# FatimaSohailll/KLT-Feature-Tracker-Acceleration-GPUs

Hardware: NVIDIA B200
Metric: tracked_features_per_s (higher is better)
Workload: dtype f32

## Files before the change

klt-feature-tracker-acceleration-gpus_b200/csrc/klt_dev.cu:

```cuda
#include <cuda_runtime.h>
#include <cub/device/device_radix_sort.cuh>
#include <cub/device/device_select.cuh>
#include <thrust/iterator/counting_iterator.h>
#include <climits>

#include <cstdarg>
#include <cstdio>
#include <cstdlib>
#include <cstring>
#include <sched.h>

#include "klt_cuda.h"

#define KLT_TRACKED         0
#define KLT_NOT_FOUND      -1
#define KLT_SMALL_DET      -2
#define KLT_MAX_ITERATIONS -3
#define KLT_OOB            -4
#define KLT_LARGE_RESIDUE  -5
#define KLT_B200_FB_INCONSISTENT -6

template <bool EXACT>
__device__ __forceinline__ float mac(float acc, float a, float b) {
  if (EXACT) return __fadd_rn(acc, __fmul_rn(a, b));
// ... 1117 lines not shown
  const unsigned char* src; int spitch;
  klt_dev_build_desc desc;
};

struct klt_dev {
  int device, num_sms;
  cudaStream_t stream;
  cudaStream_t tstream;
  cudaStream_t stream2;
  int overlap;
  cudaEvent_t ev_built[KLT_DEV_SLOTS];
  cudaEvent_t ev_read[KLT_DEV_SLOTS];
  int read_pending[KLT_DEV_SLOTS], built_pending[KLT_DEV_SLOTS];
  cudaEvent_t ev_join;
  char err[512];
  unsigned long long launches;
  int last_path, force_generic, no_fused, last_fused, track7_off;
  int W, H, L, ss;
  PyrSet set[KLT_DEV_SLOTS];
  float* arena;
  size_t arena_floats;
  int guard;
  struct Guarded { void* user; size_t bytes; } guarded[24]; int nguarded;
  float* tmp;
  unsigned char* frame;
  unsigned char* frame_buf[2]; int frame_idx;
  size_t frame_cap; int frame_pitch;
  cudaStream_t cstream;
  cudaEvent_t ev_band[KLT_BAND_EVENTS]; int band_ev_next;
  cudaEvent_t ev_frame_free[2]; int frame_busy[2];
  int band_rows, last_bands, building_slot;
  unsigned char* h_frame; size_t h_frame_cap; cudaEvent_t ev_stage_free; int stage_busy, stage_threads, last_staged;
  struct HostReg { const void* p; size_t bytes; int seen; int registered; unsigned long long stamp; } hreg[KLT_HOST_REGS];
  int reg_frames; unsigned long long reg_clock; int last_registered;
  int pdl;
  float *d_x, *d_y; int* d_val; int feat_cap; int feat_n;
  float *h_x, *h_y; int* h_val;
  int staging_busy;
  int no_track7w;
  int feat_out_host;
  unsigned char* d_rec; size_t d_rec_cap; void* h_rec; int rec_stride;
  cudaEvent_t ev_feat; int feat_pending;
  int feat_deferred; void* feat_def_dst; const void* feat_def_src; size_t feat_def_bytes;
  AffState* d_aff_st; AffState* h_aff_st; float* d_aff_tmpl; float* d_x0; int aff_cap, aff_tsz, aff_x0_cap;
  unsigned char* snap_ring; size_t snap_bytes; int snap_depth, snap_events; cudaEvent_t ev_snap[KLT_SNAP_MAX];
  int *c_val[2]; unsigned* c_idx[2]; size_t cand_cap;
  void* cub_tmp; size_t cub_bytes;
  unsigned char* fmap; size_t fmap_cap;
  int* open_slots; int open_cap;
  int* rank_list; int* sel_state;
  int no_filter; int replace_filter;
  int enforce_attr;
  unsigned* d_tile_ctr; unsigned tile_base[KLT_TILE_QUEUES];
  cudaEvent_t ev_a, ev_b; int ev_made;
  int prof_on, prof_used;
  cudaEvent_t* prof_ev;
  int* prof_kid;
  double prof_ms[KID_COUNT];
  unsigned long long prof_n[KID_COUNT];
  cudaEvent_t ev_origin;
  int trace_n; int* trace_kid; float* trace_t0; float* trace_t1;
  unsigned long long* d_live;
  FbRec* d_fb; int fb_cap, fb_n; float fb_max_error;
  PredVel* d_vel; PredRec* d_pred; int pred_cap, pred_n, vel_n;
  float* d_guess; float* h_guess; int guess_cap, guess_n, guess_slot;
  cudaEvent_t ev_guess[2]; int guess_busy[2];
  PredArgs pred;
};

static void prof_fold(klt_dev* d) {
  if (d->prof_used == 0) return;
  cudaStreamSynchronize(d->stream);
  if (d->stream2) cudaStreamSynchronize(d->stream2);
  if (d->cstream) cudaStreamSynchronize(d->cstream);
  for (int i = 0; i < d->prof_used; ++i) {
    float ms = 0.0f;
    if (cudaEventElapsedTime(&ms, d->prof_ev[2 * i], d->prof_ev[2 * i + 1]) == cudaSuccess) {
      d->prof_ms[d->prof_kid[i]] += ms;
      d->prof_n[d->prof_kid[i]] += 1;
      if (d->trace_n < TRACE_CAP) {
        float t0 = 0.0f;
        cudaEventElapsedTime(&t0, d->ev_origin, d->prof_ev[2 * i]);
        d->trace_kid[d->trace_n] = d->prof_kid[i];
        d->trace_t0[d->trace_n] = t0; d->trace_t1[d->trace_n] = t0 + ms;
        d->trace_n += 1;
      }
    }
  }
  d->prof_used = 0;
}
static int sync_all(klt_dev* d) {
  cudaError_t e = cudaStreamSynchronize(d->stream);
  if (e == cudaSuccess && d->stream2) e = cudaStreamSynchronize(d->stream2);
  if (e == cudaSuccess && d->cstream) e = cudaStreamSynchronize(d->cstream);
  d->staging_busy = 0;
  return e == cudaSuccess ? 0 : 1;
}
struct Launch {
  klt_dev* d; int slot; cudaStream_t st;
  Launch(klt_dev* d_, int kid, cudaStream_t st_ = nullptr) : d(d_), slot(-1), st(st_ ? st_ : d_->stream) {
    if (kid != KID_COPY_H2D && kid != KID_COPY_D2H) d->launches++;
    if (d->prof_on) {
      if (d->prof_used == PROF_POOL) prof_fold(d);
      slot = d->prof_used++;
      d->prof_kid[slot] = kid;
      cudaEventRecord(d->prof_ev[2 * slot], st);
// ... 136 lines not shown

static constexpr size_t KLT_GUARD_FLOATS = 1024;
static constexpr int KLT_GUARD_BYTE = 0xA5;
static cudaError_t guarded_malloc(klt_dev* d, void** out, size_t bytes) {
  if (!d->guard || d->nguarded >= (int)(sizeof(d->guarded) / sizeof(d->guarded[0]))) return cudaMalloc(out, bytes);
  const size_t gb = KLT_GUARD_FLOATS * sizeof(float), padded = (bytes + 255) / 256 * 256;
  unsigned char* base = nullptr;
  cudaError_t e = cudaMalloc(&base, padded + 2 * gb);
  if (e != cudaSuccess) return e;
  e = cudaMemset(base, KLT_GUARD_BYTE, padded + 2 * gb);
  if (e != cudaSuccess) { cudaFree(base); return e; }
  *out = base + gb;
  d->guarded[d->nguarded].user = base + gb; d->guarded[d->nguarded].bytes = bytes; d->nguarded += 1;
  return cudaSuccess;
}
template <typename T>
static cudaError_t guarded_malloc(klt_dev* d, T** out, size_t bytes) { return guarded_malloc(d, reinterpret_cast<void**>(out), bytes); }
static void guarded_free(klt_dev* d, void* p) {
  if (!p) return;
  for (int i = 0; i < d->nguarded; ++i)
    if (d->guarded[i].user == p) {
      cudaFree(static_cast<unsigned char*>(p) - KLT_GUARD_FLOATS * sizeof(float));
      d->guarded[i] = d->guarded[--d->nguarded];
      return;
    }
  cudaFree(p);
}
static void free_geometry(klt_dev* d) {
  cudaFree(d->arena); d->arena = nullptr;
  cudaFree(d->tmp); d->tmp = nullptr;
  memset(d->set, 0, sizeof(d->set));
  d->W = d->H = d->L = d->ss = 0;
}

extern "C" void klt_dev_destroy(klt_dev* d) {
  if (!d) return;
  cudaSetDevice(d->device);
  sync_all(d);
  klt_dev_forget_host_frames(d);
  free_geometry(d);
  cudaFree(d->frame_buf[0]); cudaFree(d->frame_buf[1]);
  guarded_free(d, d->d_x);
  guarded_free(d, d->d_fb);
  guarded_free(d, d->d_vel); guarded_free(d, d->d_pred); guarded_free(d, d->d_guess); cudaFreeHost(d->h_guess);
  for (int i = 0; i < 2; ++i) if (d->ev_guess[i]) cudaEventDestroy(d->ev_guess[i]);
  cudaFreeHost(d->h_x);
  for (int i = 0; i < 2; ++i) { guarded_free(d, d->c_val[i]); guarded_free(d, d->c_idx[i]); }
  cudaFree(d->cub_tmp); guarded_free(d, d->fmap); guarded_free(d, d->open_slots); guarded_free(d, d->rank_list); guarded_free(d, d->sel_state);
  if (d->ev_made) { cudaEventDestroy(d->ev_a); cudaEventDestroy(d->ev_b); }
  if (d->prof_ev) { for (int i = 0; i < 2 * PROF_POOL; ++i) cudaEventDestroy(d->prof_ev[i]); free(d->prof_ev); free(d->prof_kid);
    cudaEventDestroy(d->ev_origin); free(d->trace_kid); free(d->trace_t0); free(d->trace_t1); }
  cudaFree(d->d_live);
  cudaFree(d->d_tile_ctr);
  cudaFree(d->d_rec);
  for (int i = 0; i < KLT_DEV_SLOTS; ++i) { cudaEventDestroy(d->ev_built[i]); cudaEventDestroy(d->ev_read[i]); }
  cudaEventDestroy(d->ev_join);
  for (int i = 0; i < KLT_BAND_EVENTS; ++i) cudaEventDestroy(d->ev_band[i]);
  cudaEventDestroy(d->ev_frame_free[0]); cudaEventDestroy(d->ev_frame_free[1]);
  cudaEventDestroy(d->ev_feat);
  cudaEventDestroy(d->ev_stage_free);
  cudaFreeHost(d->h_frame);
  cudaFreeHost(d->snap_ring);
  cudaFree(d->d_aff_st); cudaFreeHost(d->h_aff_st); cudaFree(d->d_aff_tmpl); cudaFree(d->d_x0);
  for (int i = 0; i < d->snap_events; ++i) cudaEventDestroy(d->ev_snap[i]);
  cudaStreamDestroy(d->cstream);
  cudaStreamDestroy(d->stream);
  cudaStreamDestroy(d->stream2);
  free(d);
}

static int ensure_geometry(klt_dev* d, int W, int H, int L, int ss) {
  if (d->arena && d->W == W && d->H == H && d->L == L && d->ss == ss) return 0;
  if (W <= 0 || H <= 0) return fail(d, "bad image size %d x %d", W, H);
  if (L < 1 || L > KLT_DEV_MAX_LEVELS) return fail(d, "nPyramidLevels %d not in 1..%d", L, KLT_DEV_MAX_LEVELS);
  if (L > 1 && ss != 2 && ss != 4 && ss != 8 && ss != 16 && ss != 32)
    return fail(d, "Pyramid's subsampling must be either 2, 4, 8, 16, or 32");
  if (sync_all(d)) return fail(d, "stream synchronisation failed");
  memset(d->read_pending, 0, sizeof(d->read_pending));
  memset(d->built_pending, 0, sizeof(d->built_pending));
  free_geometry(d);
  d->vel_n = 0;
  size_t per_set = 0;
  int w = W, h = H;
  int ws[KLT_DEV_MAX_LEVELS], hs[KLT_DEV_MAX_LEVELS], ps[KLT_DEV_MAX_LEVELS];
  for (int l = 0; l < L; ++l) {
    ws[l] = w; hs[l] = h; ps[l] = (w + 31) / 32 * 32;
    if (w < 1 || h < 1) return fail(d, "pyramid level %d is empty (%d x %d)", l, w, h);
    per_set += 3 * (size_t)ps[l] * h;
    if (L > 1) { w /= ss; h /= ss; }
  }
  const size_t gap = d->guard ? KLT_GUARD_FLOATS : 0;
  const size_t total = KLT_DEV_SLOTS * (per_set + 3 * (size_t)L * gap) + gap;
  CU(cudaMalloc(&d->arena, total * sizeof(float) + 256));
  d->arena_floats = total;
  if (d->guard) CU(cudaMemset(d->arena, KLT_GUARD_BYTE, total * sizeof(float) + 256));
  CU(cudaMalloc(&d->tmp, (size_t)ps[0] * H * sizeof(float)));
  float* p = d->arena;
  for (int s = 0; s < KLT_DEV_SLOTS; ++s)
    for (int l = 0; l < L; ++l) {
      Level& lv = d->set[s].lv[l];
      lv.w = ws[l]; lv.h = hs[l]; lv.pitch = ps[l];
      const size_t n = (size_t)ps[l] * hs[l];
      p += gap; lv.img = p; p += n; p += gap; lv.gx = p; p += n; p += gap; lv.gy = p; p += n;
    }
  d->W = W; d->H = H; d->L = L; d->ss = ss;
  return 0;
}

extern "C" void klt_dev_set_guard(klt_dev* d, int on) {
  if (d->guard == (on ? 1 : 0)) return;
  sync_all(d);
  free_geometry(d);
  for (int i = 0; i < 2; ++i) { guarded_free(d, d->c_val[i]); guarded_free(d, d->c_idx[i]); d->c_val[i] = nullptr; d->c_idx[i] = nullptr; }
  guarded_free(d, d->rank_list); guarded_free(d, d->sel_state); d->rank_list = nullptr; d->sel_state = nullptr;
  cudaFree(d->cub_tmp); d->cub_tmp = nullptr; d->cand_cap = 0;
  guarded_free(d, d->fmap); d->fmap = nullptr; d->fmap_cap = 0;
  guarded_free(d, d->open_slots); d->open_slots = nullptr; d->open_cap = 0;
  d->guard = on ? 1 : 0;
}
extern "C" int klt_dev_check_guards(klt_dev* d, long long* damaged_words, int* first_band) {
  if (damaged_words) *damaged_words = 0;
  if (first_band) *first_band = -1;
  if (!d->guard) return 0;
  CU(cudaSetDevice(d->device));
  if (sync_all(d)) return fail(d, "stream synchronisation failed");
  unsigned* h = (unsigned*)malloc(KLT_GUARD_FLOATS * sizeof(unsigned));
  if (!h) return fail(d, "out of memory");
  const unsigned want = 0x01010101u * (unsigned)KLT_GUARD_BYTE;
  long long bad = 0;
  int first = -1, band = 0;
  auto check = [&](const float* at) -> int {
    if (cudaMemcpy(h, at, KLT_GUARD_FLOATS * sizeof(unsigned), cudaMemcpyDeviceToHost) != cudaSuccess) return 1;
    for (size_t i = 0; i < KLT_GUARD_FLOATS; ++i)
      if (h[i] != want) { bad += 1; if (first < 0) first = band; }
    band += 1;
    return 0;
  };
  int rc = 0;
  for (int s = 0; d->arena && s < KLT_DEV_SLOTS && !rc; ++s)
    for (int l = 0; l < d->L && !rc; ++l) {
      const Level& lv = d->set[s].lv[l];
      rc = check(lv.img - KLT_GUARD_FLOATS) || check(lv.gx - KLT_GUARD_FLOATS) || check(lv.gy - KLT_GUARD_FLOATS);
    }
  if (!rc && d->arena) rc = check(d->arena + d->arena_floats - KLT_GUARD_FLOATS);
  band = 1000;
  for (int i = 0; i < d->nguarded && !rc; ++i) {
    const unsigned char* u = static_cast<const unsigned char*>(d->guarded[i].user);
    rc = check(reinterpret_cast<const float*>(u - KLT_GUARD_FLOATS * sizeof(float))) ||
         check(reinterpret_cast<const float*>(u + (d->guarded[i].bytes + 255) / 256 * 256));
  }
  free(h);
  if (rc) return fail(d, "guard check: copy failed");
  if (damaged_words) *damaged_words = bad;
  if (first_band) *first_band = first;
  return 0;
}

extern "C" void* klt_dev_plane_address(const klt_dev* d, int slot, int which, int level) {
  if (!d->arena || slot < 0 || slot >= KLT_DEV_SLOTS || level < 0 || level >= d->L) return nullptr;
  const Level& lv = d->set[slot].lv[level];
  return which == 0 ? (void*)lv.img : which == 1 ? (void*)lv.gx : which == 2 ? (void*)lv.gy : nullptr;
}
extern "C" int klt_dev_poke(klt_dev* d, void* device_dst, const void* host_src, size_t bytes) {
  CU(cudaSetDevice(d->device));
  if (sync_all(d)) return fail(d, "stream synchronisation failed");
  CU(cudaMemcpy(device_dst, host_src, bytes, cudaMemcpyHostToDevice));
  return 0;
}

extern "C" int klt_dev_geometry(const klt_dev* d, int* W, int* H, int* L, int* ss) {
// ... 96 lines not shown
  { Launch l(d, KID_PYRDOWN);
    pyrdown_tile<SS, R, TXO, TYO, PY, EXACT><<<grid, NT, smem, d->stream>>>(src, spitch, W, H, t, out,
                                                                           opitch, Wout, Hout); }
  return 0;
}
template <bool EXACT>
static int pyrdown_dispatch(klt_dev* d, int ss, const float* src, int spitch, int W, int H,
                            const TapsR& t, float* out, int opitch, int Wout, int Hout, bool* done) {
  *done = true;
  const int r = t.w / 2;
  if (ss == 2 && r == 5) return launch_pyrdown<2, 5, 32, 32, 4, EXACT>(d, src, spitch, W, H, t, out, opitch, Wout, Hout);
  if (ss == 4 && r == 10) return launch_pyrdown<4, 10, 32, 16, 2, EXACT>(d, src, spitch, W, H, t, out, opitch, Wout, Hout);
  *done = false;
  return 0;
}

typedef CUresult (*EncodeTiledFn)(CUtensorMap*, CUtensorMapDataType, cuuint32_t, void*, const cuuint64_t*,
                                  const cuuint64_t*, const cuuint32_t*, const cuuint32_t*,
                                  CUtensorMapInterleave, CUtensorMapSwizzle, CUtensorMapL2promotion,
                                  CUtensorMapFloatOOBfill);
static EncodeTiledFn tma_encoder() {
  static EncodeTiledFn fn = nullptr;
  static bool tried = false;
  if (!tried) {
    tried = true;
    void* p = nullptr;
    cudaDriverEntryPointQueryResult q;
    if (cudaGetDriverEntryPoint("cuTensorMapEncodeTiled", &p, cudaEnableDefault, &q) == cudaSuccess &&
        q == cudaDriverEntryPointSuccess)
      fn = (EncodeTiledFn)p;
    cudaGetLastError();
  }
  return fn;
}
static bool make_tensor_map(CUtensorMap* m, const void* base, CUtensorMapDataType dt, int elem, int w, int h,
                            size_t pitch_bytes, int box_w, int box_h) {
  EncodeTiledFn enc = tma_encoder();
  if (!enc) return false;
  if (((uintptr_t)base & 15) || (pitch_bytes & 15) || ((box_w * elem) & 15) || box_w > 256 || box_h > 256)
    return false;
  cuuint64_t dims[2] = {(cuuint64_t)w, (cuuint64_t)h};
  cuuint64_t strides[1] = {(cuuint64_t)pitch_bytes};
  cuuint32_t box[2] = {(cuuint32_t)box_w, (cuuint32_t)box_h};
  cuuint32_t estr[2] = {1, 1};
  return enc(m, dt, 2, const_cast<void*>(base), dims, strides, box, estr, CU_TENSOR_MAP_INTERLEAVE_NONE,
             CU_TENSOR_MAP_SWIZZLE_NONE, CU_TENSOR_MAP_L2_PROMOTION_L2_128B,
             CU_TENSOR_MAP_FLOAT_OOB_FILL_NONE) == CUDA_SUCCESS;
}

static bool fused_grad_taps_ok(const TapsR& tg, const TapsR& td) {
  return tg.w == 2 * FUSED_RG + 1 && td.w == 2 * FUSED_RG + 1 && td.k[FUSED_RG] == 0.0f;
}

enum LevelShape { SHAPE_NONE = 0, SHAPE_2_5_64_32, SHAPE_2_5_64_16, SHAPE_2_5_32_16, SHAPE_4_10_32_16 };
struct FusedPlan {
  bool l0_ok;
  int shape[KLT_DEV_MAX_LEVELS];
  CUtensorMap map[KLT_DEV_MAX_LEVELS];
  int TX[KLT_DEV_MAX_LEVELS], TY[KLT_DEV_MAX_LEVELS], tiles_x[KLT_DEV_MAX_LEVELS], tiles_y[KLT_DEV_MAX_LEVELS];
  bool l0_march;
  bool chain;
  int src_plane[KLT_DEV_MAX_LEVELS], need_mul[KLT_DEV_MAX_LEVELS], need_add[KLT_DEV_MAX_LEVELS],
      made_mul[KLT_DEV_MAX_LEVELS];
};

static int level_shape_for(int ss, int r, int w, int h, int num_sms) {
  if (ss == 2 && r == 5) {
    const long px = (long)w * h;
    const long tiles_64x32 = (long)((w + 63) / 64) * ((h + 31) / 32);
    if (px >= 1500000) return SHAPE_2_5_64_32;
    if (px >= 300000) return tiles_64x32 <= 2L * num_sms ? SHAPE_2_5_64_32 : SHAPE_2_5_64_16;
    return SHAPE_2_5_32_16;
  }
  if (ss == 4 && r == 10) return SHAPE_4_10_32_16;
  return SHAPE_NONE;
}
template <int SS_, int R_, int TX_, int TY_>
struct TileShape { static constexpr int SS = SS_, R = R_, TX = TX_, TY = TY_; };
template <class F>
static auto with_shape(int shape, F f) {
  switch (shape) {
    case SHAPE_2_5_64_32: return f(TileShape<2, 5, 64, 32>());
    case SHAPE_2_5_64_16: return f(TileShape<2, 5, 64, 16>());
    case SHAPE_2_5_32_16: return f(TileShape<2, 5, 32, 16>());
    default: return f(TileShape<4, 10, 32, 16>());
  }
}

using L0GeoB = L0GeoT<48, 6, 6, 4>;
using L0GeoC = L0GeoT<40, 7, 5, 4, true>;
static int g_l0_variant = -1;
static int l0_variant() {
  if (g_l0_variant < 0) g_l0_variant = getenv("KLT_B200_L0_TILE") ? atoi(getenv("KLT_B200_L0_TILE")) : 1;
  return g_l0_variant;
}
extern "C" void klt_dev_set_l0_kernel(int variant) { g_l0_variant = variant; }
extern "C" int klt_dev_l0_kernel(void) { return l0_variant(); }
static void fused_plan(klt_dev* d, const PyrSet& S, const unsigned char* src, int spitch,
                       const klt_dev_build_desc* q, const TapsR& ts, const TapsR& tp, const TapsR& tg,
                       const TapsR& td, FusedPlan* P) {
  memset(P, 0, sizeof(*P));
  if (d->force_generic || d->no_fused || !fused_grad_taps_ok(tg, td)) return;
  const int W = q->ncols, H = q->nrows;
  const int l0_ty = l0_variant() == 1 ? L0GeoB::TY : L0Geo::TY, l0_u8h = l0_variant() == 1 ? L0GeoB::U8_H : L0Geo::U8_H;
  if (l0_variant() == 2 && q->smooth && ts.w == 2 * MarchGeo::RS + 1 &&
      make_tensor_map(&P->map[0], src, CU_TENSOR_MAP_DATA_TYPE_UINT8, 1, W, H, (size_t)spitch, MarchGeo::IN_W, MarchGeo::PU)) {
    const int nstrips = (W + MarchGeo::SWI - 1) / MarchGeo::SWI;
    const int teams = MarchGeo::CPS * d->num_sms * MarchGeo::TEAMS;
    int nseg = teams / nstrips;
    if (nseg < 1) nseg = 1;
    int seg_rows = (H + nseg - 1) / nseg;
    if (seg_rows < 16) seg_rows = 16;
    P->l0_ok = true; P->l0_march = true;
    P->TX[0] = MarchGeo::SWI; P->TY[0] = seg_rows;
    P->tiles_x[0] = nstrips; P->tiles_y[0] = (H + seg_rows - 1) / seg_rows;
  } else if (q->smooth && ts.w == 2 * L0Geo::RS + 1 &&
      make_tensor_map(&P->map[0], src, CU_TENSOR_MAP_DATA_TYPE_UINT8, 1, W, H, (size_t)spitch, L0Geo::U8_W, l0_u8h)) {
    P->l0_ok = true;
    P->TX[0] = L0Geo::TX; P->TY[0] = l0_ty;
    P->tiles_x[0] = (W + L0Geo::TX - 1) / L0Geo::TX; P->tiles_y[0] = (H + l0_ty - 1) / l0_ty;
  }
  P->need_add[0] = L0Geo::RS + L0Geo::RG;
  if (P->l0_ok && !P->l0_march && l0_variant() == 1 && q->nlevels_built > 1 && q->subsampling == 2 &&
      tp.w == 2 * NEXT_R + 1) {
    bool all = true;
    for (int l = 1; l < q->nlevels_built; ++l)
      all = all && level_shape_for(2, NEXT_R, S.lv[l].w, S.lv[l].h, d->num_sms) != SHAPE_NONE;
    CUtensorMap m0;
    if (all && make_tensor_map(&m0, src, CU_TENSOR_MAP_DATA_TYPE_UINT8, 1, W, H, (size_t)spitch, L0GeoC::U8_W,
                               L0GeoC::U8_H)) {
      P->chain = true;
      P->map[0] = m0;
      P->TY[0] = L0GeoC::TY;
      P->tiles_y[0] = (H + L0GeoC::TY - 1) / L0GeoC::TY;
      P->need_add[0] = L0GeoC::U8_H - L0GeoC::TY - (L0GeoC::RS + L0GeoC::RG + L0GeoC::XR);
    }
  }
  P->need_mul[0] = P->TY[0];
  P->made_mul[0] = P->chain ? P->TY[0] / 2 : P->TY[0];
  for (int l = 1; l < q->nlevels_built; ++l) {
    const int shape = level_shape_for(q->subsampling, tp.w / 2, S.lv[l].w, S.lv[l].h, d->num_sms);
    if (shape == SHAPE_NONE) continue;
    const Level& a = S.lv[P->chain ? l : l - 1];
    const bool ok = with_shape(shape, [&](auto s) {
      using T = decltype(s);
      P->TX[l] = T::TX; P->TY[l] = T::TY;
      if (P->chain) {
        using G = ChGeo<T::TX, T::TY>;
        P->src_plane[l] = l + 1;
        P->need_mul[l] = T::TY; P->need_add[l] = 1 - G::RN + G::SH - T::TY; P->made_mul[l] = T::TY / 2;
        return make_tensor_map(&P->map[l], a.img, CU_TENSOR_MAP_DATA_TYPE_FLOAT32, 4, a.w, a.h, (size_t)a.pitch * 4,
                               G::SW, G::SH);
      }
      using G = LvGeo<T::SS, T::R, T::TX, T::TY>;
      P->src_plane[l] = l;
      P->need_mul[l] = T::SS * T::TY; P->need_add[l] = G::YOFF + G::SH - T::SS * T::TY; P->made_mul[l] = T::TY;
      return make_tensor_map(&P->map[l], a.img, CU_TENSOR_MAP_DATA_TYPE_FLOAT32, 4, a.w, a.h, (size_t)a.pitch * 4,
                             G::SW, G::SH);
    });
    if (!ok) {
      if (P->chain) { memset(P, 0, sizeof(*P)); return; }
      continue;
    }
    P->shape[l] = shape;
    P->tiles_x[l] = (S.lv[l].w + P->TX[l] - 1) / P->TX[l];
    P->tiles_y[l] = (S.lv[l].h + P->TY[l] - 1) / P->TY[l];
  }
}

template <auto K, typename... Args>
static int launch_persistent(klt_dev* d, int kid, int nth, int smem, int ctas, int* grid, Args... args) {
  static int cps_dev[64] = {};
  int& cps = cps_dev[d->device & 63];
  if (!cps) {
    int n = 0;
    CU(cudaFuncSetAttribute(K, cudaFuncAttributeMaxDynamicSharedMemorySize, smem));
    CU(cudaOccupancyMaxActiveBlocksPerMultiprocessor(&n, K, nth, smem));
    cps = n < 1 ? 1 : n;
  }
  *grid = ctas < cps * d->num_sms ? ctas : cps * d->num_sms;
  Launch l(d, kid);
  CU(launch_k(K, dim3(*grid), dim3(nth), smem, d->stream, d->pdl != 0, args...));
  return 0;
}
struct QueueSlot {};
static constexpr QueueSlot QUEUE{};
template <class T> static T fill_queue(T a, const TileQueue&) { return a; }
static TileQueue fill_queue(QueueSlot, const TileQueue& q) { return q; }
template <auto K, typename... Args>
static int launch_tiles(klt_dev* d, int kid, int level, int nth, int smem, int tiles_x, int jr0, int jr1,
                        Args... args) {
  const int n = (jr1 - jr0) * tiles_x;
  const TileQueue q = {tiles_x, jr0 * tiles_x, jr1 * tiles_x, d->d_tile_ctr + level, d->tile_base[level]};
  int grid = 0;
  if (launch_persistent<K>(d, kid, nth, smem, n, &grid, fill_queue(args, q)...)) return 1;
  d->tile_base[level] += (unsigned)(n + grid);
  return 0;
}

template <class G, bool EXACT>
static int l0_tiles_launch(klt_dev* d, const FusedPlan& P, int W, int H, const TapsR& ts, const TapsR& tg,
                           const TapsR& td, const TapsR& tp, const Level& lv, const Level* l1, int jr0, int jr1) {
  return launch_tiles<l0_fused_kernel<G, EXACT>>(
      d, KID_L0_FUSED, 0, 256, G::SMEM, P.tiles_x[0], jr0, jr1, P.map[0], W, H, QUEUE, to_fused(ts), to_fused(tg),
      to_fused(td), lv.img, lv.gx, lv.gy, lv.pitch, to_fused(tp), l1 ? l1->img : nullptr, l1 ? l1->pitch : 0,
      l1 ? l1->w : 0, l1 ? l1->h : 0);
}
template <bool EXACT>
static int l0_fused_launch(klt_dev* d, const FusedPlan& P, int W, int H, const TapsR& ts, const TapsR& tg,
                           const TapsR& td, const TapsR& tp, const PyrSet& S, int jr0, int jr1) {
  if (jr1 <= jr0) return 0;
  if (P.l0_march) {
    using G = MarchGeo;
    const int nstrips = P.tiles_x[0], task0 = jr0 * nstrips, task1 = jr1 * nstrips;
    int grid = 0;
    return launch_persistent<l0_march_kernel<EXACT>>(
        d, KID_L0_FUSED, G::NTH, G::SMEM, (task1 - task0 + G::TEAMS - 1) / G::TEAMS, &grid, P.map[0], W, H, nstrips,
        P.TY[0], task0, task1, to_fused(ts), to_fused(tg), to_fused(td), S.lv[0].img, S.lv[0].gx, S.lv[0].gy,
        S.lv[0].pitch);
  }
  if (P.chain) return l0_tiles_launch<L0GeoC, EXACT>(d, P, W, H, ts, tg, td, tp, S.lv[0], &S.lv[1], jr0, jr1);
  if (P.TY[0] == L0GeoB::TY) return l0_tiles_launch<L0GeoB, EXACT>(d, P, W, H, ts, tg, td, tp, S.lv[0], nullptr, jr0, jr1);
  return l0_tiles_launch<L0Geo, EXACT>(d, P, W, H, ts, tg, td, tp, S.lv[0], nullptr, jr0, jr1);
}

template <bool EXACT>
static int level_launch(klt_dev* d, const FusedPlan& P, const PyrSet& S, int level, int nb, const TapsR& tp,
                        const TapsR& tg, const TapsR& td, int jr0, int jr1) {
  if (jr1 <= jr0) return 0;
  if (P.shape[level] == SHAPE_NONE) return fail(d, "level %d has no fused kernel", level);
  const Level& a = S.lv[level - 1];
  const Level& b = S.lv[level];
  const Level* nx = P.chain && level + 1 < nb ? &S.lv[level + 1] : nullptr;
  const int kid = level <= 1 ? KID_LEVEL_FUSED : level == 2 ? KID_LEVEL_FUSED_L2 : KID_LEVEL_FUSED_L3;
  const int tiles_x = P.tiles_x[level];
  return with_shape(P.shape[level], [&](auto s) {
    using T = decltype(s);
    constexpr int TX = T::TX, TY = T::TY;
    if (!P.chain)
      return launch_tiles<level_fused_kernel<T::SS, T::R, TX, TY, EXACT>>(
          d, kid, level, lv_threads<T::SS, T::R, TX, TY>(), LvGeo<T::SS, T::R, TX, TY>::SMEM, tiles_x, jr0, jr1,
          P.map[level], a.w, a.h, b.w, b.h, QUEUE, to_fused(tp), to_fused(tg), to_fused(td), b.img, b.gx, b.gy, b.pitch);
    if (nx)
      return launch_tiles<level_chain_kernel<TX, TY, true, EXACT>>(
          d, kid, level, 256, ChGeo<TX, TY>::SMEM, tiles_x, jr0, jr1, P.map[level], b.w, b.h, nx->w, nx->h, QUEUE,
          to_fused(tp), to_fused(tg), to_fused(td), b.gx, b.gy, b.pitch, nx->img, nx->pitch);
    return launch_tiles<level_chain_kernel<TX, TY, false, EXACT>>(
        d, kid, level, 256, ChGeo<TX, TY>::SMEM, tiles_x, jr0, jr1, P.map[level], b.w, b.h, 0, 0, QUEUE,
        to_fused(tp), to_fused(tg), to_fused(td), b.gx, b.gy, b.pitch, nullptr, 0);
  });
}

template <typename SrcT, bool EXACT>
static int generic_separable(klt_dev* d, const SrcT* src, int spitch, int W, int H, const TapsR& kh,
                             const TapsR& kv, int stride, float* out, int opitch, int Wout, int Hout) {
  const int off = stride / 2;
  const int tp = d->set[0].lv[0].pitch;
  dim3 b(32, 8);
  dim3 g1((Wout + 31) / 32, (H + 7) / 8);
  { Launch l(d, KID_GENERIC_H);
    conv_h_generic<SrcT, EXACT><<<g1, b, 0, d->stream>>>(src, spitch, W, H, kh, stride, off, d->tmp, tp, Wout); }
  dim3 g2((Wout + 31) / 32, (Hout + 7) / 8);
  { Launch l(d, KID_GENERIC_V);
    conv_v_generic<EXACT><<<g2, b, 0, d->stream>>>(d->tmp, tp, Wout, H, kv, stride, off, out, opitch, Hout); }
  return 0;
}

static constexpr int KLT_MAX_BANDS = 48;
struct BandFeed {
  const unsigned char* host;
  int W, H, fp;
  int nbands, next;
  int enqueued;
  bool staged;
  int end_row[KLT_MAX_BANDS];
  cudaEvent_t ev[KLT_MAX_BANDS];
};
static void feed_schedule(BandFeed* f, int mode) {
  const int H = f->H;
  f->nbands = 0;
  if (mode > 0) {
    const int rows = (mode + 63) / 64 * 64;
    int r = 0;
    while (r < H && f->nbands < KLT_MAX_BANDS - 1) {
      int take = rows;
      const int left = H - r;
      if (left > rows && left < rows + rows / 2) take = left - rows / 2;
      if (take > left) take = left;
      r += take;
      f->end_row[f->nbands++] = r;
    }
    if (r < H) f->end_row[f->nbands++] = H;
  } else if (mode < 0 && (long)f->W * H >= 4L * 1000 * 1000) {
    static float frac[8] = {0.6f};
    static int nfrac = 1;
    static bool parsed = false;
    if (!parsed) {
      parsed = true;
      const char* e = getenv("KLT_B200_BAND_FRACS");
      if (e && *e) {
        nfrac = 0;
        while (*e && nfrac < 8) {
          char* end = nullptr;
// ... 119 lines not shown
  if (pageable && host_frame_register(d, f->host, bytes)) pageable = false;
  f->staged = d->stage_threads > 0 && pageable;
  d->last_staged = f->staged ? 1 : 0;
  if (f->staged) {
    if (d->h_frame_cap < bytes) {
      if (sync_all(d)) return fail(d, "stream synchronisation failed");
      cudaFreeHost(d->h_frame); d->h_frame = nullptr; d->h_frame_cap = 0;
      CU(cudaHostAlloc(&d->h_frame, bytes, cudaHostAllocDefault));
      d->h_frame_cap = bytes;
      d->stage_busy = 0;
    }
    if (d->stage_busy) { CU(cudaEventSynchronize(d->ev_stage_free)); d->stage_busy = 0; }
    return 0;
  }
  for (int b = 0; b < f->nbands; ++b)
    if (feed_enqueue_band(d, f, b)) return 1;
  return 0;
}
static int feed_wait(klt_dev* d, BandFeed* f, bool all, int* rows) {
  do {
    if (f->next >= f->enqueued && feed_enqueue_band(d, f, f->next)) return 1;
    CU(cudaStreamWaitEvent(d->stream, f->ev[f->next], 0));
    f->next += 1;
  } while (all && f->next < f->nbands);
  *rows = f->end_row[f->next - 1];
  return 0;
}

template <bool EXACT>
static int build_impl(klt_dev* d, PyrSet& S, const unsigned char* src, int spitch,
                      const klt_dev_build_desc* q, BandFeed* feed) {
  const int W = q->ncols, H = q->nrows;
  bool tiled_all = true, done = false;
  const int nb = q->nlevels_built;
  TapsR ts, tp;
  memset(&ts, 0, sizeof(ts)); memset(&tp, 0, sizeof(tp));
  if (q->smooth) ts = reversed(q->smooth_taps.gauss, q->smooth_taps.gauss_width);
  if (nb > 1) tp = reversed(q->pyramid_taps.gauss, q->pyramid_taps.gauss_width);
  const TapsR tg = reversed(q->grad_taps.gauss, q->grad_taps.gauss_width);
  const TapsR td = reversed(q->grad_taps.deriv, q->grad_taps.deriv_width);
  FusedPlan P;
  d->last_fused = 0;
  d->last_bands = 0;
  fused_plan(d, S, src, spitch, q, ts, tp, tg, td, &P);
  bool all_fused = P.l0_ok;
  for (int l = 1; l < nb; ++l) all_fused = all_fused && P.shape[l] != SHAPE_NONE;

  if (all_fused) {
    int rows_done[KLT_DEV_MAX_LEVELS] = {0};
    int valid[KLT_DEV_MAX_LEVELS + 1] = {0};
    auto plane_h = [&](int p) { return p == 0 ? H : S.lv[p - 1].h; };
    valid[0] = feed ? 0 : H;
    if (feed && feed_enqueue_copies(d, feed)) return 1;
    do {
      if (feed && feed_wait(d, feed, false, &valid[0])) return 1;
      for (int l = 0; l < nb; ++l) {
        const int sp = P.src_plane[l];
        int j = rows_done[l];
        while (j < P.tiles_y[l]) {
          int need = P.need_mul[l] * (j + 1) + P.need_add[l];
          if (need > plane_h(sp)) need = plane_h(sp);
          if (need > valid[sp]) break;
          ++j;
        }
        if (l == 0 ? l0_fused_launch<EXACT>(d, P, W, H, ts, tg, td, tp, S, rows_done[0], j)
                   : level_launch<EXACT>(d, P, S, l, nb, tp, tg, td, rows_done[l], j))
          return 1;
        rows_done[l] = j;
        if (l + 1 < nb) {
          const int np = P.src_plane[l + 1];
          valid[np] = P.made_mul[l] * j < plane_h(np) ? P.made_mul[l] * j : plane_h(np);
        }
      }
    } while (valid[0] < H);
    if (feed) {
      d->last_bands = feed->nbands;
      CU(cudaEventRecord(d->ev_frame_free[d->frame_idx], d->stream));
      d->frame_busy[d->frame_idx] = 1;
    }
    for (int l = 0; l < nb; ++l)
      if (rows_done[l] != P.tiles_y[l]) return fail(d, "banded build left level %d incomplete", l);
    d->last_fused = nb;
    d->last_path = 1;
    return 0;
  }

  if (feed) {
    int rows = 0;
    feed->nbands = 1; feed->end_row[0] = H;
    if (feed_enqueue_copies(d, feed) || feed_wait(d, feed, true, &rows)) return 1;
    d->last_bands = 1;
  }
  int grad_from = 0;
  if (P.l0_ok) {
    if (l0_fused_launch<EXACT>(d, P, W, H, ts, tg, td, tp, S, 0, P.tiles_y[0])) return 1;
    grad_from = 1;
  }
  d->last_fused = grad_from;
  if (grad_from == 1) {
  } else if (q->smooth) {
    done = false;
    if (!d->force_generic)
      if (smooth_u8_dispatch<EXACT>(d, src, spitch, W, H, ts, S.lv[0].img, S.lv[0].pitch, &done)) return 1;
    if (!done) {
      tiled_all = false;
      if (generic_separable<unsigned char, EXACT>(d, src, spitch, W, H, ts, ts, 1, S.lv[0].img,
                                                  S.lv[0].pitch, W, H)) return 1;
    }
  } else {
    dim3 b(32, 8), g((W + 31) / 32, (H + 7) / 8);
    Launch l(d, KID_U8_TO_F32);
    u8_to_f32_kernel<<<g, b, 0, d->stream>>>(src, spitch, W, H, S.lv[0].img, S.lv[0].pitch);
  }
  if (feed) {
    CU(cudaEventRecord(d->ev_frame_free[d->frame_idx], d->stream));
    d->frame_busy[d->frame_idx] = 1;
  }
  bool grads_done[KLT_DEV_MAX_LEVELS] = {false};
  grads_done[0] = (grad_from == 1);
  for (int l = 1; l < nb; ++l) {
    const Level& a = S.lv[l - 1];
    const Level& b = S.lv[l];
    if (P.shape[l] != SHAPE_NONE) {
      if (level_launch<EXACT>(d, P, S, l, nb, tp, tg, td, 0, P.tiles_y[l])) return 1;
      grads_done[l] = true; d->last_fused += 1;
      continue;
    }
    done = false;
    if (!d->force_generic)
      if (pyrdown_dispatch<EXACT>(d, q->subsampling, a.img, a.pitch, a.w, a.h, tp, b.img, b.pitch,
                                  b.w, b.h, &done)) return 1;
    if (!done) {
      tiled_all = false;
      if (generic_separable<float, EXACT>(d, a.img, a.pitch, a.w, a.h, tp, tp, q->subsampling,
// ... 946 lines not shown
```

klt-feature-tracker-acceleration-gpus_b200/csrc/klt_fused.cuh:

```cuda
#pragma once

#include <cuda.h>

__device__ __forceinline__ unsigned smem_u32(const void* p) {
  return (unsigned)__cvta_generic_to_shared(p);
}
__device__ __forceinline__ void mbar_init(unsigned long long* bar, unsigned count) {
  asm volatile("mbarrier.init.shared::cta.b64 [%0], %1;" ::"r"(smem_u32(bar)), "r"(count) : "memory");
  asm volatile("fence.mbarrier_init.release.cluster;" ::: "memory");
}
__device__ __forceinline__ void mbar_expect_tx(unsigned long long* bar, unsigned bytes) {
  asm volatile("mbarrier.arrive.expect_tx.shared::cta.b64 _, [%0], %1;" ::"r"(smem_u32(bar)), "r"(bytes)
               : "memory");
}
__device__ __forceinline__ void mbar_wait(unsigned long long* bar, unsigned phase) {
  asm volatile(
      "{\n\t"
      ".reg .pred P1;\n\t"
      "KLT_WAIT:\n\t"
      "mbarrier.try_wait.parity.shared::cta.b64 P1, [%0], %1;\n\t"
      "@P1 bra KLT_DONE;\n\t"
      "bra KLT_WAIT;\n\t"
      "KLT_DONE:\n\t"
      "}" ::"r"(smem_u32(bar)), "r"(phase)
// ... 601 lines not shown

template <int TX, int TY>
struct ChGeo {
  static constexpr int RG = FUSED_RG, RN = NEXT_R;
  static constexpr int SW = TX + 12, SH = TY + 2 * RN - 1;
  static constexpr int HP = TX + 4, GH = TY + 2 * RG;
  static constexpr int NP = TX / 2 + 4;
  static_assert(SW >= TX + 2 * RN - 1 && (SW / 4) % 2 == 1 && (HP / 4) % 2 == 1, "box width / odd chunk pitches");
  static_assert(RN - 1 - RG >= 0, "the gradient rows lie inside the box");
  static constexpr int OFF_SRC = 0;
  static constexpr int OFF_HD = OFF_SRC + SW * SH * 4;
  static constexpr int OFF_HG = OFF_HD + GH * HP * 4;
  static constexpr int OFF_N = OFF_HG + GH * HP * 4;
  static constexpr int OFF_BAR = OFF_N + SH * NP * 4;
  static constexpr int SMEM = OFF_BAR + 16;
};

template <int TX, int TY, bool NX, bool EXACT>
__global__ void __launch_bounds__(256, 4)
level_chain_kernel(const __grid_constant__ CUtensorMap map, int W, int H, int Wn, int Hn,
                   const __grid_constant__ TileQueue q, TapsF tp, TapsF tg, TapsF td, float* __restrict__ out_gx,
                   float* __restrict__ out_gy, int opitch, float* __restrict__ out_next, int npitch) {
  using G = ChGeo<TX, TY>;
  extern __shared__ __align__(128) unsigned char smem_raw[];
  const float* sL = reinterpret_cast<const float*>(smem_raw + G::OFF_SRC);
  const float* sLg = sL + (G::RN - 1 - G::RG) * G::SW;
  float* sHd = reinterpret_cast<float*>(smem_raw + G::OFF_HD);
  float* sHg = reinterpret_cast<float*>(smem_raw + G::OFF_HG);
  float* sN = reinterpret_cast<float*>(smem_raw + G::OFF_N);
  constexpr int PY = (TX / 4) * (TY / 2) <= 128 ? 2 : ((TX / 4) * (TY / 4) <= 128 ? 4 : 8);
  auto border = [&](int x0, int y0) { return (x0 < 8) || (y0 < 8) || (x0 + TX + 8 > W) || (y0 + TY + 8 > H); };
  tile_queue<TX, TY, true>(
      q, &map, smem_raw + G::OFF_SRC, G::SW * G::SH * 4, smem_raw + G::OFF_BAR, border,
      [&](int x0, int y0) { return make_int2(x0 - 4, y0 + 1 - G::RN); },
      [&](int x0, int y0, bool border) {
        if (border) {
          stage_hgrad<EXACT, true, TX, G::GH, G::SW, G::HP>(sLg, sHd, sHg, tg, td, x0, W);
          if (NX) stage_hnext<EXACT, true, TX, G::SH, G::SW, G::NP>(sL, sN, tp, x0, W);
        } else {
          stage_hgrad<EXACT, false, TX, G::GH, G::SW, G::HP>(sLg, sHd, sHg, tg, td, x0, W);
          if (NX) stage_hnext<EXACT, false, TX, G::SH, G::SW, G::NP>(sL, sN, tp, x0, W);
        }
      },
      [&](int x0, int y0, bool border) {
        if (border) {
          stage_vgrad_both<EXACT, true, TX, TY, PY, G::HP>(sHd, sHg, tg, td, out_gx, out_gy, opitch, x0, y0, W, H);
          if (NX) stage_vnext<EXACT, true, TX, TY, G::NP>(sN, tp, out_next, npitch, x0, y0, H, Wn, Hn);
        } else {
          stage_vgrad_both<EXACT, false, TX, TY, PY, G::HP>(sHd, sHg, tg, td, out_gx, out_gy, opitch, x0, y0, W, H);
          if (NX) stage_vnext<EXACT, false, TX, TY, G::NP>(sN, tp, out_next, npitch, x0, y0, H, Wn, Hn);
        }
      });
}
```

Measured before the change: 59.01 million.

## Fuse coarse pyramid levels into one persistent tail kernel with row dependencies

Adds a persistent level_tail_kernel that builds every coarse pyramid level (1..n) in one launch. A host-side schedule interleaves tile rows across levels, and per-row release/acquire counters let a tile wait only on the source rows it reads, with a TMA prefetch of the next tile overlapping the back half of the current one. The aim is to remove per-level launch overhead and the serialization between small coarse-level kernels, which underfill the GPU. The cost is more complexity, spin-waiting on device-side dependency counters, and a fixed cap on tile rows.

Measured after the change: 54.89 million, median of 6. 0.93x the previous value.

```diff
diff --git a/klt-feature-tracker-acceleration-gpus_b200/csrc/klt_dev.cu b/klt-feature-tracker-acceleration-gpus_b200/csrc/klt_dev.cu
--- a/klt-feature-tracker-acceleration-gpus_b200/csrc/klt_dev.cu
+++ b/klt-feature-tracker-acceleration-gpus_b200/csrc/klt_dev.cu
@@ -1193,6 +1193,7 @@
   int no_filter; int replace_filter;
   int enforce_attr;
   unsigned* d_tile_ctr; unsigned tile_base[KLT_TILE_QUEUES];
+  unsigned* d_tail_rows; unsigned tail_epoch; int tail_sig[2 * KLT_DEV_MAX_LEVELS + 1]; int tail_open;
   cudaEvent_t ev_a, ev_b; int ev_made;
   int prof_on, prof_used;
   cudaEvent_t* prof_ev;
@@ -1435,6 +1436,7 @@
     cudaEventDestroy(d->ev_origin); free(d->trace_kid); free(d->trace_t0); free(d->trace_t1); }
   cudaFree(d->d_live);
   cudaFree(d->d_tile_ctr);
+  guarded_free(d, d->d_tail_rows);
   cudaFree(d->d_rec);
   for (int i = 0; i < KLT_DEV_SLOTS; ++i) { cudaEventDestroy(d->ev_built[i]); cudaEventDestroy(d->ev_read[i]); }
   cudaEventDestroy(d->ev_join);
@@ -1499,6 +1501,7 @@
   cudaFree(d->cub_tmp); d->cub_tmp = nullptr; d->cand_cap = 0;
   guarded_free(d, d->fmap); d->fmap = nullptr; d->fmap_cap = 0;
   guarded_free(d, d->open_slots); d->open_slots = nullptr; d->open_cap = 0;
+  guarded_free(d, d->d_tail_rows); d->d_tail_rows = nullptr;
   d->guard = on ? 1 : 0;
 }
 extern "C" int klt_dev_check_guards(klt_dev* d, long long* damaged_words, int* first_band) {
@@ -1701,7 +1704,6 @@
   return tg.w == 2 * FUSED_RG + 1 && td.w == 2 * FUSED_RG + 1 && td.k[FUSED_RG] == 0.0f;
 }
 
-enum LevelShape { SHAPE_NONE = 0, SHAPE_2_5_64_32, SHAPE_2_5_64_16, SHAPE_2_5_32_16, SHAPE_4_10_32_16 };
 struct FusedPlan {
   bool l0_ok;
   int shape[KLT_DEV_MAX_LEVELS];
@@ -1709,6 +1711,7 @@
   int TX[KLT_DEV_MAX_LEVELS], TY[KLT_DEV_MAX_LEVELS], tiles_x[KLT_DEV_MAX_LEVELS], tiles_y[KLT_DEV_MAX_LEVELS];
   bool l0_march;
   bool chain;
+  bool tail;
   int src_plane[KLT_DEV_MAX_LEVELS], need_mul[KLT_DEV_MAX_LEVELS], need_add[KLT_DEV_MAX_LEVELS],
       made_mul[KLT_DEV_MAX_LEVELS];
 };
@@ -1815,6 +1818,11 @@
     P->tiles_x[l] = (S.lv[l].w + P->TX[l] - 1) / P->TX[l];
     P->tiles_y[l] = (S.lv[l].h + P->TY[l] - 1) / P->TY[l];
   }
+  if (P->chain && q->nlevels_built >= 3) {
+    int rows = 0;
+    for (int l = 1; l < q->nlevels_built; ++l) rows += P->tiles_y[l];
+    P->tail = rows <= TAIL_MAX_ROWS;
+  }
 }
 
 template <auto K, typename... Args>
@@ -1898,6 +1906,89 @@
         d, kid, level, 256, ChGeo<TX, TY>::SMEM, tiles_x, jr0, jr1, P.map[level], b.w, b.h, 0, 0, QUEUE,
         to_fused(tp), to_fused(tg), to_fused(td), b.gx, b.gy, b.pitch, nullptr, 0);
   });
+}
+
+static int tail_begin(klt_dev* d, const FusedPlan& P, int nb) {
+  int sig[2 * KLT_DEV_MAX_LEVELS + 1] = {nb};
+  for (int l = 1; l < nb; ++l) { sig[2 * l - 1] = P.tiles_x[l]; sig[2 * l] = P.tiles_y[l]; }
+  if (!d->d_tail_rows) {
+    CU(guarded_malloc(d, &d->d_tail_rows, TAIL_MAX_ROWS * sizeof(unsigned)));
+    CU(cudaDeviceSynchronize());
+    d->tail_sig[0] = -1;
+  }
+  if (d->tail_open || memcmp(sig, d->tail_sig, sizeof(sig)) != 0) {
+    CU(cudaMemsetAsync(d->d_tail_rows, 0, TAIL_MAX_ROWS * sizeof(unsigned), d->stream));
+    memcpy(d->tail_sig, sig, sizeof(sig));
+    d->tail_epoch = 0;
+  }
+  d->tail_open = 1;
+  return 0;
+}
+static constexpr int TAIL_CPS = 4;
+template <bool EXACT>
+static int tail_launch(klt_dev* d, const FusedPlan& P, const PyrSet& S, int nb, const TapsR& tp, const TapsR& tg,
+                       const TapsR& td, const int* r0, const int* r1) {
+  TailArgs a;
+  memset(&a, 0, sizeof(a));
+  int off[KLT_DEV_MAX_LEVELS] = {0};
+  for (int l = 1; l < nb; ++l) {
+    if (l + 1 < nb) off[l + 1] = off[l] + P.tiles_y[l];
+    const Level& b = S.lv[l];
+    const Level* nx = l + 1 < nb ? &S.lv[l + 1] : nullptr;
+    TailLevel& L = a.lv[l];
+    a.map[l] = P.map[l];
+    L.shape = P.shape[l]; L.tiles_x = P.tiles_x[l];
+    L.W = b.w; L.H = b.h; L.Wn = nx ? nx->w : 0; L.Hn = nx ? nx->h : 0; L.opitch = b.pitch; L.npitch = nx ? nx->pitch : 0;
+    L.gx = b.gx; L.gy = b.gy; L.next = nx ? nx->img : nullptr;
+    L.rows = nx ? d->d_tail_rows + off[l] : nullptr;
+    L.dep = l >= 2 ? d->d_tail_rows + off[l - 1] : nullptr;
+    L.dep_target = l >= 2 ? (d->tail_epoch + 1) * (unsigned)P.tiles_x[l - 1] : 0u;
+  }
+  auto deps = [&](int l, int j, int* k0, int* k1) {
+    const int made = P.made_mul[l - 1];
+    int lo = P.TY[l] * j + 1 - NEXT_R, hi = P.need_mul[l] * (j + 1) + P.need_add[l];
+    if (lo < 0) lo = 0;
+    if (hi > S.lv[l].h) hi = S.lv[l].h;
+    *k0 = lo / made;
+    *k1 = (hi + made - 1) / made < P.tiles_y[l - 1] ? (hi + made - 1) / made : P.tiles_y[l - 1];
+  };
+  int nxt[KLT_DEV_MAX_LEVELS];
+  for (int l = 1; l < nb; ++l) nxt[l] = r0[l];
+  long end_tile[TAIL_MAX_ROWS];
+  const long lag = (long)TAIL_CPS * d->num_sms;
+  long ntiles = 0;
+  auto ready = [&](int l, int* k0, int* k1) {
+    if (nxt[l] >= r1[l]) return 0;
+    deps(l, nxt[l], k0, k1);
+    if (*k1 > nxt[l - 1]) return 0;
+    return *k1 <= r0[l - 1] || ntiles - end_tile[off[l - 1] + *k1 - 1] >= lag ? 2 : 1;
+  };
+  for (;;) {
+    int l = 0, k0 = 0, k1 = 0;
+    for (int c = nb - 1; c >= 2 && !l; --c)
+      if (ready(c, &k0, &k1) == 2) l = c;
+    if (!l && nxt[1] < r1[1]) l = 1;
+    for (int c = 2; c < nb && !l; ++c)
+      if (ready(c, &k0, &k1)) l = c;
+    if (!l) break;
+    if (a.nent == TAIL_MAX_ROWS) return fail(d, "level_tail_kernel: more than %d tile rows", TAIL_MAX_ROWS);
+    TailEntry& e = a.ent[a.nent++];
+    e.start = ntiles; e.level = (unsigned char)l; e.row = (unsigned short)nxt[l];
+    e.dep0 = (unsigned short)(l >= 2 ? k0 : 0); e.ndep = (unsigned char)(l >= 2 ? k1 - k0 : 0);
+    ntiles += P.tiles_x[l];
+    end_tile[off[l] + nxt[l]] = ntiles;
+    nxt[l] += 1;
+  }
+  for (int l = 1; l < nb; ++l)
+    if (nxt[l] != r1[l]) return fail(d, "level_tail_kernel: level %d row %d reads rows not scheduled yet", l, nxt[l]);
+  if (a.nent == 0) return 0;
+  a.counter = d->d_tile_ctr + 1; a.base = d->tile_base[1]; a.ntiles = (int)ntiles;
+  int grid = 0;
+  if (launch_persistent<level_tail_kernel<EXACT>>(d, KID_LEVEL_FUSED, 256, TAIL_SMEM, (int)ntiles, &grid, a,
+                                                  to_fused(tp), to_fused(tg), to_fused(td)))
+    return 1;
+  d->tile_base[1] += (unsigned)(ntiles + grid);
+  return 0;
 }
 
 template <typename SrcT, bool EXACT>
@@ -2123,8 +2214,10 @@
     auto plane_h = [&](int p) { return p == 0 ? H : S.lv[p - 1].h; };
     valid[0] = feed ? 0 : H;
     if (feed && feed_enqueue_copies(d, feed)) return 1;
+    if (P.tail && tail_begin(d, P, nb)) return 1;
     do {
       if (feed && feed_wait(d, feed, false, &valid[0])) return 1;
+      int r0[KLT_DEV_MAX_LEVELS], r1[KLT_DEV_MAX_LEVELS];
       for (int l = 0; l < nb; ++l) {
         const int sp = P.src_plane[l];
         int j = rows_done[l];
@@ -2134,8 +2227,9 @@
           if (need > valid[sp]) break;
           ++j;
         }
+        r0[l] = rows_done[l]; r1[l] = j;
         if (l == 0 ? l0_fused_launch<EXACT>(d, P, W, H, ts, tg, td, tp, S, rows_done[0], j)
-                   : level_launch<EXACT>(d, P, S, l, nb, tp, tg, td, rows_done[l], j))
+                   : !P.tail && level_launch<EXACT>(d, P, S, l, nb, tp, tg, td, rows_done[l], j))
           return 1;
         rows_done[l] = j;
         if (l + 1 < nb) {
@@ -2143,6 +2237,7 @@
           valid[np] = P.made_mul[l] * j < plane_h(np) ? P.made_mul[l] * j : plane_h(np);
         }
       }
+      if (P.tail && tail_launch<EXACT>(d, P, S, nb, tp, tg, td, r0, r1)) return 1;
     } while (valid[0] < H);
     if (feed) {
       d->last_bands = feed->nbands;
@@ -2151,6 +2246,7 @@
     }
     for (int l = 0; l < nb; ++l)
       if (rows_done[l] != P.tiles_y[l]) return fail(d, "banded build left level %d incomplete", l);
+    if (P.tail) { d->tail_epoch += 1; d->tail_open = 0; }
     d->last_fused = nb;
     d->last_path = 1;
     return 0;
diff --git a/klt-feature-tracker-acceleration-gpus_b200/csrc/klt_fused.cuh b/klt-feature-tracker-acceleration-gpus_b200/csrc/klt_fused.cuh
--- a/klt-feature-tracker-acceleration-gpus_b200/csrc/klt_fused.cuh
+++ b/klt-feature-tracker-acceleration-gpus_b200/csrc/klt_fused.cuh
@@ -677,3 +677,159 @@
         }
       });
 }
+
+enum LevelShape { SHAPE_NONE = 0, SHAPE_2_5_64_32, SHAPE_2_5_64_16, SHAPE_2_5_32_16, SHAPE_4_10_32_16 };
+static constexpr int TAIL_MAX_ROWS = 256;
+using TailG = ChGeo<64, 32>;
+static constexpr int TAIL_SMEM = TailG::OFF_BAR + 32;
+template <int TX, int TY>
+__device__ __forceinline__ unsigned char* tail_back_bufs(unsigned char* smem) {
+  using G = ChGeo<TX, TY>;
+  static_assert(G::SW * G::SH <= TailG::SW * TailG::SH && G::OFF_BAR - G::OFF_HD <= TailG::OFF_BAR - TailG::OFF_HD,
+                "tail buffers");
+  return smem + (TailG::OFF_HD - G::OFF_HD);
+}
+struct TailLevel {
+  int shape;
+  int tiles_x, W, H, Wn, Hn, opitch, npitch;
+  float *gx, *gy, *next;
+  unsigned* rows;
+  const unsigned* dep;
+  unsigned dep_target;
+};
+struct TailEntry {
+  unsigned start;
+  unsigned short row, dep0;
+  unsigned char level, ndep;
+};
+struct TailArgs {
+  CUtensorMap map[KLT_DEV_MAX_LEVELS];
+  TailLevel lv[KLT_DEV_MAX_LEVELS];
+  unsigned* counter; unsigned base;
+  int ntiles, nent;
+  TailEntry ent[TAIL_MAX_ROWS];
+};
+
+__device__ __forceinline__ void red_release_add(unsigned* p, unsigned v) {
+  asm volatile("red.release.gpu.global.add.u32 [%0], %1;" ::"l"(p), "r"(v) : "memory");
+}
+__device__ __forceinline__ bool tail_rows_ready(const TailArgs& a, const TailEntry& e) {
+  const TailLevel& L = a.lv[e.level];
+  if (!L.dep) return true;
+  for (int r = e.dep0; r < e.dep0 + e.ndep; ++r)
+    if ((int)(ld_acquire_u32(L.dep + r) - L.dep_target) < 0) return false;
+  return true;
+}
+
+template <bool EXACT, int TX, int TY>
+__device__ __forceinline__ void tail_front(unsigned char* smem, const TailLevel& L, const TapsF& tp, const TapsF& tg,
+                                           const TapsF& td, int x0, int y0) {
+  using G = ChGeo<TX, TY>;
+  const float* sL = reinterpret_cast<const float*>(smem + G::OFF_SRC);
+  const float* sLg = sL + (G::RN - 1 - G::RG) * G::SW;
+  unsigned char* bufs = tail_back_bufs<TX, TY>(smem);
+  float* sHd = reinterpret_cast<float*>(bufs + G::OFF_HD);
+  float* sHg = reinterpret_cast<float*>(bufs + G::OFF_HG);
+  float* sN = reinterpret_cast<float*>(bufs + G::OFF_N);
+  const int W = L.W, H = L.H;
+  const bool nx = L.next != nullptr;
+  if ((x0 < 8) || (y0 < 8) || (x0 + TX + 8 > W) || (y0 + TY + 8 > H)) {
+    stage_hgrad<EXACT, true, TX, G::GH, G::SW, G::HP>(sLg, sHd, sHg, tg, td, x0, W);
+    if (nx) stage_hnext<EXACT, true, TX, G::SH, G::SW, G::NP>(sL, sN, tp, x0, W);
+  } else {
+    stage_hgrad<EXACT, false, TX, G::GH, G::SW, G::HP>(sLg, sHd, sHg, tg, td, x0, W);
+    if (nx) stage_hnext<EXACT, false, TX, G::SH, G::SW, G::NP>(sL, sN, tp, x0, W);
+  }
+}
+template <bool EXACT, int TX, int TY>
+__device__ __forceinline__ void tail_back(unsigned char* smem, const TailLevel& L, const TapsF& tp, const TapsF& tg,
+                                          const TapsF& td, int x0, int y0) {
+  using G = ChGeo<TX, TY>;
+  const unsigned char* bufs = tail_back_bufs<TX, TY>(smem);
+  const float* sHd = reinterpret_cast<const float*>(bufs + G::OFF_HD);
+  const float* sHg = reinterpret_cast<const float*>(bufs + G::OFF_HG);
+  const float* sN = reinterpret_cast<const float*>(bufs + G::OFF_N);
+  constexpr int PY = (TX / 4) * (TY / 2) <= 128 ? 2 : ((TX / 4) * (TY / 4) <= 128 ? 4 : 8);
+  const int W = L.W, H = L.H;
+  const bool nx = L.next != nullptr;
+  if ((x0 < 8) || (y0 < 8) || (x0 + TX + 8 > W) || (y0 + TY + 8 > H)) {
+    stage_vgrad_both<EXACT, true, TX, TY, PY, G::HP>(sHd, sHg, tg, td, L.gx, L.gy, L.opitch, x0, y0, W, H);
+    if (nx) stage_vnext<EXACT, true, TX, TY, G::NP>(sN, tp, L.next, L.npitch, x0, y0, H, L.Wn, L.Hn);
+  } else {
+    stage_vgrad_both<EXACT, false, TX, TY, PY, G::HP>(sHd, sHg, tg, td, L.gx, L.gy, L.opitch, x0, y0, W, H);
+    if (nx) stage_vnext<EXACT, false, TX, TY, G::NP>(sN, tp, L.next, L.npitch, x0, y0, H, L.Wn, L.Hn);
+  }
+}
+__device__ __forceinline__ int tail_tx(int shape) { return shape == SHAPE_2_5_32_16 ? 32 : 64; }
+__device__ __forceinline__ int tail_ty(int shape) { return shape == SHAPE_2_5_64_32 ? 32 : 16; }
+
+template <bool EXACT>
+__global__ void __launch_bounds__(256, 4)
+level_tail_kernel(const __grid_constant__ TailArgs a, TapsF tp, TapsF tg, TapsF td) {
+  extern __shared__ __align__(128) unsigned char smem_raw[];
+  unsigned char* sched = smem_raw + TailG::OFF_BAR;
+  unsigned long long* bar = reinterpret_cast<unsigned long long*>(sched);
+  volatile int* s_tile = reinterpret_cast<volatile int*>(sched + 8);
+  volatile int* s_ent = reinterpret_cast<volatile int*>(sched + 12);
+  volatile int* s_loaded = reinterpret_cast<volatile int*>(sched + 16);
+  const int tid = threadIdx.x;
+  int e = 0;
+  auto load = [&](int t, int ei) {
+    const TailEntry& en = a.ent[ei];
+    const int l = en.level, shape = a.lv[l].shape;
+    const int tx = tail_tx(shape), ty = tail_ty(shape);
+    const int x0 = (t - (int)en.start) * tx, y0 = en.row * ty;
+    asm volatile("fence.proxy.async.global;" ::: "memory");
+    mbar_expect_tx(bar, (unsigned)((tx + 12) * (ty + 2 * NEXT_R - 1) * 4));
+    tma_load_2d(smem_raw, &a.map[l], x0 - 4, y0 + 1 - NEXT_R, bar);
+  };
+  auto claim = [&]() {
+    if (tid == 0) {
+      const int t = (int)(atomicAdd(a.counter, 1u) - a.base);
+      *s_tile = t;
+      if (t < a.ntiles) {
+        while (e + 1 < a.nent && (int)a.ent[e + 1].start <= t) ++e;
+        *s_ent = e;
+        const bool ready = tail_rows_ready(a, a.ent[e]);
+        *s_loaded = ready;
+        if (ready) load(t, e);
+      }
+    }
+  };
+  if (tid == 0) {
+    mbar_init(bar, 1);
+    for (int l = 1; l < KLT_DEV_MAX_LEVELS && a.lv[l].tiles_x > 0; ++l)
+      asm volatile("prefetch.tensormap [%0];" ::"l"(reinterpret_cast<unsigned long long>(&a.map[l])) : "memory");
+  }
+  pdl_wait();
+  claim();
+  __syncthreads();
+  unsigned phase = 0;
+  for (;;) {
+    const int t = *s_tile;
+    if (t >= a.ntiles) break;
+    const int ei = *s_ent;
+    const TailEntry& en = a.ent[ei];
+    const int l = en.level;
+    const TailLevel& L = a.lv[l];
+    const int shape = L.shape;
+    const int x0 = (t - (int)en.start) * tail_tx(shape), y0 = en.row * tail_ty(shape);
+    if (tid == 0 && !*s_loaded) {
+      while (!tail_rows_ready(a, en)) __nanosleep(64);
+      load(t, ei);
+    }
+    mbar_wait(bar, phase);
+    phase ^= 1;
+    if (shape == SHAPE_2_5_64_32) tail_front<EXACT, 64, 32>(smem_raw, L, tp, tg, td, x0, y0);
+    else if (shape == SHAPE_2_5_64_16) tail_front<EXACT, 64, 16>(smem_raw, L, tp, tg, td, x0, y0);
+    else tail_front<EXACT, 32, 16>(smem_raw, L, tp, tg, td, x0, y0);
+    __syncthreads();
+    claim();
+    if (shape == SHAPE_2_5_64_32) tail_back<EXACT, 64, 32>(smem_raw, L, tp, tg, td, x0, y0);
+    else if (shape == SHAPE_2_5_64_16) tail_back<EXACT, 64, 16>(smem_raw, L, tp, tg, td, x0, y0);
+    else tail_back<EXACT, 32, 16>(smem_raw, L, tp, tg, td, x0, y0);
+    __syncthreads();
+    if (tid == 0 && L.rows) red_release_add(L.rows + en.row, 1u);
+  }
+  pdl_launch_dependents();
+}
```
